# EveryVoiceTTS/EveryVoice

Measured on AMD Instinct MI355X. Metric: hifigan_v1_infer_audio_samples_per_sec, higher is better.
Workload: dtype bf16; 1 GPU; HiFiGAN-V1 generator inference, mel[32,80,768] -> wav[32,1,196608] per GPU, 1 replica(s), upstream N(0,0.01) init, weight norm folded; global_batch=32, frames=768, parallelism=replicas x1

## Files before the change

### everyvoice_amd/csrc/common.h

```cpp
#pragma once

#include <hip/hip_runtime.h>
#include <stdint.h>

#include <cstdio>
#include <cstdlib>
#include <string>

#include "evmi.h"

namespace evmi {

constexpr int kMaxDevices = 16;
inline int device_slot() {
  int d = 0;
  if (hipGetDevice(&d) != hipSuccess || d < 0 || d >= kMaxDevices) return 0;
  return d;
}


void set_error(const std::string& msg);
int fail(int code, const std::string& msg);

#define EVMI_HIP_CHECK(expr)                                                                   \
  do {                                                                                         \
    hipError_t _e = (expr);                                                                    \
    if (_e != hipSuccess) {                                                                    \
      return ::evmi::fail(EVMI_ERR_HIP, std::string(#expr) + ": " + hipGetErrorString(_e));    \
    }                                                                                          \
  } while (0)

#define EVMI_LAUNCH_CHECK(what)                                                                \
  do {                                                                                         \
    hipError_t _e = hipGetLastError();                                                         \
    if (_e != hipSuccess) {                                                                    \
      return ::evmi::fail(EVMI_ERR_HIP, std::string(what) + " launch: " + hipGetErrorString(_e)); \
    }                                                                                          \
  } while (0)

constexpr int kMaxLdsKernels = 256;
inline int ensure_dynamic_lds(const void* kernel, size_t bytes) {
  struct Record { const void* kernel; size_t bytes; };
  static thread_local Record records[kMaxDevices][kMaxLdsKernels];
  static thread_local int n_records[kMaxDevices] = {};
  int d = -1;
  if (hipGetDevice(&d) != hipSuccess || d >= kMaxDevices) d = -1;
  Record* r = nullptr;
  if (d >= 0) {
    for (int i = 0; i < n_records[d] && !r; ++i)
      if (records[d][i].kernel == kernel) r = &records[d][i];
    if (r && bytes <= r->bytes) return EVMI_OK;
  }
  const hipError_t e = hipFuncSetAttribute(kernel, hipFuncAttributeMaxDynamicSharedMemorySize, (int)bytes);
  if (e != hipSuccess)
    return fail(EVMI_ERR_HIP, "hipFuncSetAttribute(MaxDynamicSharedMemorySize, " + std::to_string(bytes) + "): " + hipGetErrorString(e));
  if (r) r->bytes = bytes;
  else if (d >= 0 && n_records[d] < kMaxLdsKernels) records[d][n_records[d]++] = Record{kernel, bytes};
  return EVMI_OK;
}

template <typename... Params, typename... Args>
inline int launch_with_lds(void (*kernel)(Params...), dim3 grid, dim3 block, size_t lds, hipStream_t stream, Args&&... args) {
  if (int rc = ensure_dynamic_lds((const void*)kernel, lds)) return rc;
  hipLaunchKernelGGL(kernel, grid, block, lds, stream, static_cast<Args&&>(args)...);
  return EVMI_OK;
}

inline int env_int(const char* name, int dflt) {
  const char* e = getenv(name);
  return e ? atoi(e) : dflt;
}
inline bool env_set(const char* name) { return getenv(name) != nullptr; }

typedef __bf16 bf16_t;
typedef __bf16 bf16x8 __attribute__((ext_vector_type(8)));
typedef __bf16 bf16x4 __attribute__((ext_vector_type(4)));
typedef float f32x16 __attribute__((ext_vector_type(16)));
typedef float f32x4 __attribute__((ext_vector_type(4)));
typedef unsigned int u32x4 __attribute__((ext_vector_type(4)));

__device__ __forceinline__ float lrelu(float v, float slope) { return v > 0.f ? v : v * slope; }

__device__ __forceinline__ u32x4 swap_quads_bf16(u32x4 d) {
  const auto r0 = __builtin_amdgcn_permlane32_swap(d[0], d[2], false, false);
  const auto r1 = __builtin_amdgcn_permlane32_swap(d[1], d[3], false, false);
  u32x4 o;
  o[0] = r0[0];
  o[2] = r0[1];
  o[1] = r1[0];
  o[3] = r1[1];
  return o;
}
__device__ __forceinline__ unsigned pack_bf16x2(float lo, float hi) {
  typedef __bf16 bf16x2_t __attribute__((ext_vector_type(2)));
  bf16x2_t pk;
  pk[0] = (bf16_t)lo;
  pk[1] = (bf16_t)hi;
  return __builtin_bit_cast(unsigned, pk);
}
__device__ __forceinline__ float bf16_lo(unsigned d) { return __builtin_bit_cast(float, d << 16); }
__device__ __forceinline__ float bf16_hi(unsigned d) { return __builtin_bit_cast(float, d & 0xffff0000u); }

__device__ __forceinline__ void lds_barrier() {
  asm volatile("s_waitcnt lgkmcnt(0)\n\ts_barrier" ::: "memory");
}

__device__ __forceinline__ void lds_dma_barrier() {
  asm volatile("s_waitcnt vmcnt(0)" ::: "memory");
  __syncthreads();
}

template <int MT, int NT, int KSTEPS, int NTAPS, int A_TAP_STRIDE, int A_MT_STRIDE, int B_NT_STRIDE, int PRIO = 0>
__device__ __forceinline__ void mma_tap_group(const bf16_t* __restrict__ Arow, const bf16_t* __restrict__ Brow,
                                              int b_tap_stride, f32x16 (&acc)[MT][NT]) {
  constexpr int N = NTAPS * KSTEPS;
  bf16x8 af[2][MT], bfr[2][NT];
  auto load = [&](int kk, int buf) {
    const int jj = kk / KSTEPS, ks = kk % KSTEPS;
#pragma unroll
    for (int mt = 0; mt < MT; ++mt)
      af[buf][mt] = *reinterpret_cast<const bf16x8*>(Arow + jj * A_TAP_STRIDE + mt * A_MT_STRIDE + ks * 16);
#pragma unroll
    for (int nt = 0; nt < NT; ++nt)
      bfr[buf][nt] = *reinterpret_cast<const bf16x8*>(Brow + jj * b_tap_stride + nt * B_NT_STRIDE + ks * 16);
  };
  load(0, 0);
#pragma unroll
  for (int kk = 0; kk < N; ++kk) {
    const int cur = kk & 1;
    if (kk + 1 < N) load(kk + 1, cur ^ 1);
    if (PRIO) __builtin_amdgcn_s_setprio(1);
#pragma unroll
    for (int mt = 0; mt < MT; ++mt)
#pragma unroll
      for (int nt = 0; nt < NT; ++nt)
        acc[mt][nt] = __builtin_amdgcn_mfma_f32_32x32x16_bf16(af[cur][mt], bfr[cur][nt], acc[mt][nt], 0, 0, 0);
    if (PRIO) __builtin_amdgcn_s_setprio(0);
  }
}

__device__ __forceinline__ bf16x4 lrelu4_bf16(f32x4 f, float slope) {
  const f32x4 m = f * slope;
  bf16x4 r;
#pragma unroll
  for (int e = 0; e < 4; ++e) r[e] = (bf16_t)fmaxf(f[e], m[e]);
  return r;
}
__device__ __forceinline__ bf16x8 lrelu8_bf16(bf16x8 x, float slope) {
  f32x4 lo, hi;
#pragma unroll
  for (int e = 0; e < 4; ++e) { lo[e] = (float)x[e]; hi[e] = (float)x[4 + e]; }
  const f32x4 ml = lo * slope, mh = hi * slope;
  bf16x8 r;
#pragma unroll
  for (int e = 0; e < 4; ++e) { r[e] = (bf16_t)fmaxf(lo[e], ml[e]); r[4 + e] = (bf16_t)fmaxf(hi[e], mh[e]); }
  return r;
}

inline uint16_t f32_to_bf16_bits(float f) {
  uint32_t u;
  __builtin_memcpy(&u, &f, 4);
  if ((u & 0x7fffffffu) > 0x7f800000u) return (uint16_t)((u >> 16) | 0x40);
  u += 0x7fffu + ((u >> 16) & 1u);
  return (uint16_t)(u >> 16);
}

__device__ __forceinline__ float ordered_sum_strided(const float* __restrict__ p, long long stride, int n, float acc = 0.f) {
  int s = 0;
  for (; s + 16 <= n; s += 16) {
    float v[16];
#pragma unroll
    for (int u = 0; u < 16; ++u) v[u] = p[(long long)(s + u) * stride];
#pragma unroll
    for (int u = 0; u < 16; ++u) acc += v[u];
  }
  for (; s < n; s += 8) {
    float v[8];
#pragma unroll
    for (int u = 0; u < 8; ++u) v[u] = p[(long long)min(s + u, n - 1) * stride];
#pragma unroll
    for (int u = 0; u < 8; ++u) acc = s + u < n ? acc + v[u] : acc;
  }
  return acc;
}


__device__ __forceinline__ float silu_grad(float z) {
#pragma clang fp contract(off)
  const float sg = 1.f / (1.f + expf(-z));
  return sg * (1.f + z * (1.f - sg));
}
__device__ __forceinline__ float silu_value(float v) {
#pragma clang fp contract(off)
  return v / (1.f + expf(-v));
}

struct SeedArg {
  unsigned long long value;
  const unsigned long long* base;
  __device__ __forceinline__ unsigned long long get() const { return base ? ((value + *base) & 0x7FFFFFFFFFFFFFFFull) : value; }
};

__device__ __forceinline__ unsigned dropout_hash(unsigned long long seed, unsigned j_lo, unsigned j_hi) {
  const unsigned k0 = (unsigned)seed * 0x9E3779B1u + 0x7F4A7C15u;
  unsigned k1 = (unsigned)(seed >> 32) ^ (k0 >> 15);
  k1 = k1 * 0x85EBCA6Bu + 0xC2B2AE35u;
  unsigned h = j_lo ^ k0;
  h += j_hi * 0x27D4EB2Fu;
  h ^= h >> 16;
  h *= 0x7FEB352Du;
  h ^= k1;
  h ^= h >> 15;
  h *= 0x846CA68Bu;
  h ^= h >> 16;
  return h;
}
__device__ __forceinline__ float dropout_u16(unsigned h, unsigned odd) { return (float)(odd ? h >> 16 : h & 0xFFFFu) * (1.0f / 65536.0f); }
__device__ __forceinline__ float uniform01(unsigned long long seed, unsigned long long i) {
  const unsigned long long j = i >> 1;
  return dropout_u16(dropout_hash(seed, (unsigned)j, (unsigned)(j >> 32)), (unsigned)i & 1u);
}
__device__ __forceinline__ void dropout_pair(unsigned long long seed, unsigned j, float& u_even, float& u_odd) {
  const unsigned h = dropout_hash(seed, j, 0u);
  u_even = dropout_u16(h, 0u);
  u_odd = dropout_u16(h, 1u);
}


__device__ __forceinline__ float wave_sum_dpp(float v) {
  v += __builtin_bit_cast(float, __builtin_amdgcn_mov_dpp(__builtin_bit_cast(int, v), 0xB1, 0xF, 0xF, true));
  v += __builtin_bit_cast(float, __builtin_amdgcn_mov_dpp(__builtin_bit_cast(int, v), 0x4E, 0xF, 0xF, true));
  v += __builtin_bit_cast(float, __builtin_amdgcn_mov_dpp(__builtin_bit_cast(int, v), 0x141, 0xF, 0xF, true));
  v += __builtin_bit_cast(float, __builtin_amdgcn_mov_dpp(__builtin_bit_cast(int, v), 0x140, 0xF, 0xF, true));
  const int b = __builtin_bit_cast(int, v);
  const float r0 = __builtin_bit_cast(float, __builtin_amdgcn_readlane(b, 0)), r1 = __builtin_bit_cast(float, __builtin_amdgcn_readlane(b, 16));
  const float r2 = __builtin_bit_cast(float, __builtin_amdgcn_readlane(b, 32)), r3 = __builtin_bit_cast(float, __builtin_amdgcn_readlane(b, 48));
  return (r0 + r1) + (r2 + r3);
}

template <int CTRL>
__device__ __forceinline__ double dpp_move_f64(double v) {
  const long long b = __builtin_bit_cast(long long, v);
  const int lo = __builtin_amdgcn_mov_dpp((int)(b & 0xFFFFFFFFll), CTRL, 0xF, 0xF, true);
  const int hi = __builtin_amdgcn_mov_dpp((int)(b >> 32), CTRL, 0xF, 0xF, true);
  return __builtin_bit_cast(double, ((long long)hi << 32) | (long long)(unsigned)lo);
}
__device__ __forceinline__ double wave_sum_dpp_f64(double v) {
  v += dpp_move_f64<0xB1>(v);
  v += dpp_move_f64<0x4E>(v);
  v += dpp_move_f64<0x141>(v);
  v += dpp_move_f64<0x140>(v);
  const long long b = __builtin_bit_cast(long long, v);
  const int lo = (int)(b & 0xFFFFFFFFll), hi = (int)(b >> 32);
  double r[4];
#pragma unroll
  for (int q = 0; q < 4; ++q) {
    const int l = __builtin_amdgcn_readlane(lo, 16 * q), h = __builtin_amdgcn_readlane(hi, 16 * q);
    r[q] = __builtin_bit_cast(double, ((long long)h << 32) | (long long)(unsigned)l);
  }
  return (r[0] + r[1]) + (r[2] + r[3]);
}

__device__ __forceinline__ void wait_vmcnt_le(int n) {
  n = __builtin_amdgcn_readfirstlane(n);
#define EVMI_VMCASE(N) case N: asm volatile("s_waitcnt vmcnt(" #N ")" ::: "memory"); break;
  switch (n) {
    EVMI_VMCASE(0) EVMI_VMCASE(1) EVMI_VMCASE(2) EVMI_VMCASE(3) EVMI_VMCASE(4) EVMI_VMCASE(5) EVMI_VMCASE(6)
    EVMI_VMCASE(7) EVMI_VMCASE(8) EVMI_VMCASE(9) EVMI_VMCASE(10) EVMI_VMCASE(11) EVMI_VMCASE(12) EVMI_VMCASE(13)
    EVMI_VMCASE(14) EVMI_VMCASE(15) EVMI_VMCASE(16) EVMI_VMCASE(17) EVMI_VMCASE(18) EVMI_VMCASE(19) EVMI_VMCASE(20)
    EVMI_VMCASE(21) EVMI_VMCASE(22) EVMI_VMCASE(23) EVMI_VMCASE(24) EVMI_VMCASE(25) EVMI_VMCASE(26) EVMI_VMCASE(27)
    EVMI_VMCASE(28) EVMI_VMCASE(29) EVMI_VMCASE(30) EVMI_VMCASE(31) EVMI_VMCASE(32) EVMI_VMCASE(33) EVMI_VMCASE(34)
    EVMI_VMCASE(35) EVMI_VMCASE(36) EVMI_VMCASE(37) EVMI_VMCASE(38) EVMI_VMCASE(39) EVMI_VMCASE(40) EVMI_VMCASE(41)
    EVMI_VMCASE(42) EVMI_VMCASE(43) EVMI_VMCASE(44) EVMI_VMCASE(45) EVMI_VMCASE(46) EVMI_VMCASE(47) EVMI_VMCASE(48)
    EVMI_VMCASE(49) EVMI_VMCASE(50) EVMI_VMCASE(51) EVMI_VMCASE(52) EVMI_VMCASE(53) EVMI_VMCASE(54) EVMI_VMCASE(55)
    EVMI_VMCASE(56) EVMI_VMCASE(57) EVMI_VMCASE(58) EVMI_VMCASE(59) EVMI_VMCASE(60) EVMI_VMCASE(61) EVMI_VMCASE(62)
    default: asm volatile("s_waitcnt vmcnt(63)" ::: "memory"); break;
  }
#undef EVMI_VMCASE
}


int launch_mha_fwd_bf16_plain(const float* qkv, const int* lens, float* out, float* lse_or_null, int B, int T, int D, int heads,
                              hipStream_t s);

}
```

### everyvoice_amd/csrc/conv_tc_dma_kernel.h

```cpp
#pragma once

#include <type_traits>

#include "conv_tc_mfma.h"

namespace evmi {

static __device__ __attribute__((aligned(128))) bf16_t g_conv_dma_zero_row[64];

typedef __attribute__((address_space(3))) void lds_void_t;
typedef __attribute__((address_space(1))) const void glb_void_t;
__device__ __forceinline__ void lds_dma_b128(const void* g, void* l) {
  __builtin_amdgcn_global_load_lds((glb_void_t*)g, (lds_void_t*)l, 16, 0, 0);
}

template <int CIN_, int KS_, int MAXDIL_, int DBG_ = 0, int VAR_ = 0, int WN_ = 4>
struct ConvDmaCfg {
  static constexpr int CIN = CIN_, KS = KS_, MAXDIL = MAXDIL_, DBG = DBG_, VAR = VAR_;
  static constexpr int KC = 64, BM = 128, WM = 2, WN = WN_, MT = 2, NT = 2, BN = WN * NT * 32;
  static constexpr int NTHREADS = WM * WN * 64, NWAVES = WM * WN;
  static constexpr int NCHUNK = CIN / KC, NSTEP = NCHUNK * KS;
  static constexpr int R_MAX = BN + (KS - 1) * MAXDIL;
  static constexpr int X_PIECES = (R_MAX + 7) / 8;
  static constexpr int X_BYTES = X_PIECES * 1024;
  static constexpr int A_PIECES = BM / 8;
  static constexpr int A_BYTES = A_PIECES * 1024;
  static constexpr int OS = BM + 8;
  static constexpr size_t LDS_MAIN = size_t(X_BYTES) + 2 * A_BYTES;
  static constexpr size_t LDS_OUT = size_t(BN) * OS * 2;
  static constexpr size_t LDS = LDS_MAIN > LDS_OUT ? LDS_MAIN : LDS_OUT;
  static constexpr int X_VEC_PER_THREAD = (X_PIECES * 64 + NTHREADS - 1) / NTHREADS;
  static_assert(CIN % KC == 0, "channel chunking");
  static_assert((WN == 4 ? 2 : 1) * LDS <= 160 * 1024, "two workgroups per CU (one for the 16-wave form)");
  static_assert(A_PIECES % NWAVES == 0 || NWAVES == 16, "weight pieces per wave");
};

template <class C>
__global__ __launch_bounds__(C::NTHREADS, 4) void conv_tc_dma_kernel(ConvTcArgs a) {
  static_assert(C::NWAVES == 2 || C::NWAVES == 4 || C::NWAVES == 8 || C::NWAVES == 16, "2, 4, 8 or 16 waves");
  extern __shared__ __attribute__((aligned(1024))) char smem[];
  char* Xs = smem;
  char* As = smem + C::X_BYTES;

  const int tid = threadIdx.x;
  const int lane = tid & 63;
  const int wave = __builtin_amdgcn_readfirstlane(tid >> 6);
  const int wm = wave / C::WN, wn = wave % C::WN;
  const int r0 = blockIdx.x * C::BN;
  const int b = blockIdx.y;
  const int mtile = blockIdx.z;
  const int m0 = mtile * C::BM;

  const bf16_t* __restrict__ xb = a.x + (long long)b * a.x_batch_stride;
  const bf16_t* __restrict__ wb = a.w + (long long)mtile * C::NSTEP * C::BM * C::KC;

  int n_stamp = 0;
  auto stamp = [&]() {
    if (C::DBG && a.timeline && blockIdx.x == 5 && blockIdx.y == 1 && blockIdx.z == 0 && lane == 0 && n_stamp < 120)
      a.timeline[wave * 128 + n_stamp++] = (long long)__builtin_readcyclecounter();
  };
  stamp();

  const int h = lane >> 5;
  const long long ob = (long long)b * a.out_batch_stride;
  long long flat_nt[C::NT];
  bool row_ok[C::NT];
#pragma unroll
  for (int nt = 0; nt < C::NT; ++nt) {
    const int r = r0 + wn * (C::NT * 32) + nt * 32 + (lane & 31);
    flat_nt[nt] = (long long)r * a.out_row_stride + m0 + wm * (C::MT * 32) + 8 * h + a.out_shift;
    row_ok[nt] = r < a.n_rows;
  }
  auto vec_index = [&](int nt, int co) -> long long {
    const long long f = flat_nt[nt] + co;
    return (row_ok[nt] && f >= 0 && f + 8 <= a.out_limit) ? f : -1;
  };
  auto swap_quads = [](u32x4 d) -> u32x4 { return swap_quads_bf16(d); };

  f32x16 acc[C::MT][C::NT];
#pragma unroll
  for (int mt = 0; mt < C::MT; ++mt)
#pragma unroll
    for (int q = 0; q < 4; ++q) {
      const f32x4 bv = *reinterpret_cast<const f32x4*>(a.bias + m0 + wm * (C::MT * 32) + mt * 32 + 8 * q + 4 * h);
#pragma unroll
      for (int nt = 0; nt < C::NT; ++nt)
#pragma unroll
        for (int i = 0; i < 4; ++i) acc[mt][nt][4 * q + i] = bv[i];
    }
  const int rows_needed = C::BN + (C::KS - 1) * a.dil;
  const int x_pieces = (rows_needed + 7) >> 3;
  const float pre = a.pre_slope;

  auto issue_a = [&](int step) {
    const bf16_t* src = wb + (long long)step * (C::BM * C::KC) + lane * 8;
    char* dst = As + (step & 1) * C::A_BYTES;
    if (C::VAR & 1024) {
      if (wave < C::NWAVES / 2) {
#pragma unroll
        for (int i = 0; i < 2 * C::A_PIECES / C::NWAVES; ++i) {
          const int p = wave + i * (C::NWAVES / 2);
          lds_dma_b128(src + p * 512, dst + p * 1024);
        }
      }
      return;
    }
#pragma unroll
    for (int i = 0; i < (C::A_PIECES + C::NWAVES - 1) / C::NWAVES; ++i) {
      const int p = wave + i * C::NWAVES;
      if (p < C::A_PIECES) lds_dma_b128(src + p * 512, dst + p * 1024);
    }
  };
  auto issue_x = [&](int chunk) {
    const int slot = lane & 7;
    for (int p = wave; p < x_pieces; p += C::NWAVES) {
      const int row = p * 8 + (lane >> 3);
      const int rr = r0 - a.pad + row;
      const int c8 = slot ^ ((row >> 1) & 7);
      const bf16_t* src = (row < rows_needed && rr >= 0 && rr < a.t_in) ? xb + (long long)rr * C::CIN + chunk * C::KC + c8 * 8
                                                                        : g_conv_dma_zero_row + slot * 8;
      lds_dma_b128(src, Xs + p * 1024);
    }
  };

  const int row_a = wm * (C::MT * 32) + (lane & 31);
  const int s_a = (row_a >> 1) & 7;
  int off_a[4];
#pragma unroll
  for (int ks = 0; ks < 4; ++ks) off_a[ks] = row_a * 128 + (((2 * ks + h) ^ s_a) << 4);

  auto mma_step = [&](const char* Ab, int tap, int next_step) {
    const int q = wn * (C::NT * 32) + (lane & 31) + tap * a.dil;
    const int s_b = (q >> 1) & 7;
    int off_b[4];
#pragma unroll
    for (int ks = 0; ks < 4; ++ks) off_b[ks] = q * 128 + (((2 * ks + h) ^ s_b) << 4);
    bf16x8 af[2][C::MT], bfr[2][C::NT];
    auto load = [&](int ks, int buf) {
#pragma unroll
      for (int mt = 0; mt < C::MT; ++mt) af[buf][mt] = *reinterpret_cast<const bf16x8*>(Ab + off_a[ks] + mt * (32 * 128));
#pragma unroll
      for (int nt = 0; nt < C::NT; ++nt) bfr[buf][nt] = *reinterpret_cast<const bf16x8*>(Xs + off_b[ks] + nt * (32 * 128));
    };
    load(0, 0);
#pragma unroll
    for (int ks = 0; ks < 4; ++ks) {
      const int cur = (C::VAR & 32) ? 0 : (ks & 1);
      if (ks + 1 < 4 && !(C::VAR & 32)) load(ks + 1, cur ^ 1);
      if ((C::VAR & 2048) && ks == 0 && next_step >= 0) issue_a(next_step);
      if (C::VAR & 2) __builtin_amdgcn_sched_barrier(0);
      if (C::VAR & 4) __builtin_amdgcn_s_setprio(1);
#pragma unroll
      for (int mt = 0; mt < C::MT; ++mt)
#pragma unroll
        for (int nt = 0; nt < C::NT; ++nt)
          acc[mt][nt] = __builtin_amdgcn_mfma_f32_32x32x16_bf16(af[cur][mt], bfr[cur][nt], acc[mt][nt], 0, 0, 0);
      if (C::VAR & 4) __builtin_amdgcn_s_setprio(0);
      if (C::VAR & 2) __builtin_amdgcn_sched_barrier(0);
    }
  };
  if ((C::VAR & 1) && wave >= C::NWAVES / 2) __builtin_amdgcn_s_setprio(1);

  issue_x(0);
  issue_a(0);
#pragma unroll 1
  for (int chunk = 0; chunk < C::NCHUNK; ++chunk) {
    if (chunk > 0 && !(C::VAR & 64)) {
      __syncthreads();
      issue_x(chunk);
    }
    if (pre != 1.f && !((C::VAR & 64) && chunk > 0)) {
      lds_dma_barrier();
#pragma unroll
      for (int i = 0; i < C::X_VEC_PER_THREAD; ++i) {
        const int v = tid + i * C::NTHREADS;
        if (v < x_pieces * 64) {
          bf16x8 val = *reinterpret_cast<const bf16x8*>(Xs + v * 16);
#pragma unroll
          for (int e = 0; e < 8; ++e) {
            const float f = (float)val[e];
            val[e] = (bf16_t)fmaxf(f, f * pre);
          }
          *reinterpret_cast<bf16x8*>(Xs + v * 16) = val;
        }
      }
    }
    stamp();
#pragma unroll 1
    for (int tap = 0; tap < C::KS; ++tap) {
      const int step = chunk * C::KS + tap;
      if (!(C::VAR & (16 | 256)) || step == 0) lds_dma_barrier();
      stamp();
      const bool more = step + 1 < C::NSTEP && !(C::VAR & (16 | 512));
      if (more && !(C::VAR & 2048)) issue_a(step + 1);
      mma_step(As + (step & 1) * C::A_BYTES, tap, (more && (C::VAR & 2048)) ? step + 1 : -1);
      stamp();
    }
  }

  if (C::VAR & 128) {
    float sacc = 0.f;
#pragma unroll
    for (int mt = 0; mt < C::MT; ++mt)
#pragma unroll
      for (int nt = 0; nt < C::NT; ++nt)
#pragma unroll
        for (int r = 0; r < 16; ++r) sacc += acc[mt][nt][r];
    if (sacc == 12345.678f) a.out[0] = (bf16_t)sacc;
    return;
  }
  stamp();
  if (a.res || a.mask) {
    __syncthreads();
    bf16_t* Os = reinterpret_cast<bf16_t*>(smem);
#pragma unroll
    for (int mt = 0; mt < C::MT; ++mt)
#pragma unroll
      for (int q = 0; q < 4; ++q) {
        const int c = wm * C::MT * 32 + mt * 32 + 8 * q + 4 * h;
#pragma unroll
        for (int nt = 0; nt < C::NT; ++nt) {
          const int n = wn * C::NT * 32 + nt * 32 + (lane & 31);
          bf16x4 pk;
#pragma unroll
          for (int i = 0; i < 4; ++i) pk[i] = (bf16_t)acc[mt][nt][4 * q + i];
          *reinterpret_cast<bf16x4*>(Os + n * C::OS + c) = pk;
        }
      }
    __syncthreads();
    const float scale = a.out_scale, post = a.post_slope;
    constexpr int VPR = C::BM / 8;
    constexpr int OPT = C::BN * VPR / C::NTHREADS;
    constexpr int EB = 4;
    static_assert(C::BN * VPR % C::NTHREADS == 0 && OPT % EB == 0, "epilogue tiling");
    auto flat_index = [&](int v) -> long long {
      const int n = v / VPR, c8 = v % VPR;
      const int r = r0 + n;
      const long long flat = (long long)r * a.out_row_stride + m0 + c8 * 8 + a.out_shift;
      return (r >= a.n_rows || flat < 0 || flat >= a.out_limit) ? -1 : flat;
    };
    const float mslope = a.mask_slope;
    auto body = [&](auto has_acc, auto has_res, auto has_mask) {
      constexpr bool ACC = decltype(has_acc)::value, RES = decltype(has_res)::value, MSK = decltype(has_mask)::value;
#pragma unroll
      for (int i0 = 0; i0 < OPT; i0 += EB) {
        bf16x8 rv[EB], pv[EB], mv[EB];
#pragma unroll
        for (int i = 0; i < EB; ++i) {
          const long long flat = flat_index(tid + (i0 + i) * C::NTHREADS);
          const long long safe = flat < 0 ? 0 : flat;
          if (RES) rv[i] = *reinterpret_cast<const bf16x8*>(a.res + ob + safe);
          if (ACC) pv[i] = *reinterpret_cast<const bf16x8*>(a.out + ob + safe);
          if (MSK) mv[i] = *reinterpret_cast<const bf16x8*>(a.mask + ob + safe);
        }
#pragma unroll
        for (int i = 0; i < EB; ++i) {
          const int v = tid + (i0 + i) * C::NTHREADS;
          const long long flat = flat_index(v);
          const int n = v / VPR, c8 = v % VPR;
          const bf16x8 o = *reinterpret_cast<const bf16x8*>(Os + n * C::OS + c8 * 8);
          float f[8];
#pragma unroll
          for (int e = 0; e < 8; ++e) f[e] = (float)o[e];
          if (MSK) {
#pragma unroll
            for (int e = 0; e < 8; ++e) f[e] = (float)mv[i][e] > 0.f ? f[e] : f[e] * mslope;
          }
          if (RES) {
#pragma unroll
            for (int e = 0; e < 8; ++e) f[e] += (float)rv[i][e];
          }
#pragma unroll
          for (int e = 0; e < 8; ++e) f[e] *= scale;
          if (ACC) {
#pragma unroll
            for (int e = 0; e < 8; ++e) f[e] += (float)pv[i][e];
          }
          bf16x8 res;
#pragma unroll
          for (int e = 0; e < 8; ++e) res[e] = (bf16_t)(post != 1.f ? lrelu(f[e], post) : f[e]);
          if (flat >= 0) *reinterpret_cast<bf16x8*>(a.out + ob + flat) = res;
        }
      }
    };
    using T_ = std::integral_constant<bool, true>;
    using F_ = std::integral_constant<bool, false>;
    if (a.mask) {
      if (a.res) body(F_{}, T_{}, T_{});
      else body(F_{}, F_{}, T_{});
    } else if (a.accumulate) body(T_{}, T_{}, F_{});
    else body(F_{}, T_{}, F_{});
  } else {
    const float scale = a.out_scale, post = a.post_slope;
    auto body = [&](auto has_acc) {
      constexpr bool ACC = decltype(has_acc)::value;
#pragma unroll
      for (int mt = 0; mt < C::MT; ++mt) {
        u32x4 pv[C::NT][2];
        if (ACC) {
#pragma unroll
          for (int nt = 0; nt < C::NT; ++nt)
#pragma unroll
            for (int p2 = 0; p2 < 2; ++p2) {
              const long long f = vec_index(nt, mt * 32 + 16 * p2);
              pv[nt][p2] = *reinterpret_cast<const u32x4*>(a.out + ob + (f < 0 ? 0 : f));
            }
        }
#pragma unroll
        for (int nt = 0; nt < C::NT; ++nt)
#pragma unroll
          for (int p2 = 0; p2 < 2; ++p2) {
            float f[8];
#pragma unroll
            for (int e = 0; e < 8; ++e) f[e] = acc[mt][nt][8 * p2 + e] * scale;
            if (ACC) {
              const u32x4 d = swap_quads(pv[nt][p2]);
#pragma unroll
              for (int w = 0; w < 4; ++w) {
                f[2 * w] += __builtin_bit_cast(float, d[w] << 16);
                f[2 * w + 1] += __builtin_bit_cast(float, d[w] & 0xffff0000u);
              }
            }
            u32x4 o;
#pragma unroll
            for (int w = 0; w < 4; ++w) {
              const float lo = post != 1.f ? lrelu(f[2 * w], post) : f[2 * w];
              const float hi = post != 1.f ? lrelu(f[2 * w + 1], post) : f[2 * w + 1];
              typedef __bf16 bf16x2_t __attribute__((ext_vector_type(2)));
              bf16x2_t pk;
              pk[0] = (bf16_t)lo;
              pk[1] = (bf16_t)hi;
              o[w] = __builtin_bit_cast(unsigned, pk);
            }
            o = swap_quads(o);
            const long long fo = vec_index(nt, mt * 32 + 16 * p2);
            if (fo >= 0) *reinterpret_cast<u32x4*>(a.out + ob + fo) = o;
          }
      }
    };
    if (a.accumulate) body(std::integral_constant<bool, true>{});
    else body(std::integral_constant<bool, false>{});
  }
  stamp();
}

template <class C>
static ConvTcLaunch make_conv_dma_launch(const char* name) {
  ConvTcLaunch l;
  l.kernel = conv_tc_dma_kernel<C>;
  l.bm = C::BM;
  l.bn = C::BN;
  l.kc = C::KC;
  l.threads = C::NTHREADS;
  l.lds_bytes = C::LDS;
  l.name = name;
  l.wlayout = 1;
  return l;
}

}
```

### everyvoice_amd/csrc/conv_tc_mfma.hip

```cpp
#include "conv_tc_dma_kernel.h"
#include "conv_tc_kernel.h"

namespace evmi {

struct ConvTcEntry {
  int c_in, ks, max_dil, kc;
  ConvTcLaunch launch;
};

template <class C>
static ConvTcEntry make_entry(const char* name) {
  ConvTcEntry e;
  e.c_in = C::CIN;
  e.ks = C::KS;
  e.max_dil = C::MAXDIL;
  e.kc = C::KC;
  e.launch = make_conv_tc_launch<C>(name);
  return e;
}

#define EVMI_CONV_TC_TABLE(X)                                                        \
                                                         \
  X(80, 80, 128, 128, 2, 2, 7, 1, 1)                                                 \
                          \
  X(512, 64, 128, 256, 2, 4, 2, 1, 1)                                                \
  X(256, 64, 128, 256, 2, 4, 2, 1, 1)                                                \
  X(128, 64, 128, 256, 2, 4, 2, 1, 1)                                                \
  X(64, 64, 64, 256, 1, 8, 2, 2, 1)                                                  \
                                 \
  X(256, 64, 128, 256, 2, 4, 3, 1, 5)                                                \
  X(256, 64, 128, 256, 2, 4, 7, 1, 5)                                                \
  X(256, 64, 128, 256, 2, 4, 11, 1, 5)                                               \
  X(128, 64, 128, 256, 2, 4, 3, 1, 5)                                                \
  X(128, 64, 128, 256, 2, 4, 7, 1, 5)                                                \
  X(128, 64, 128, 256, 2, 4, 11, 1, 5)                                               \
  X(64, 64, 64, 256, 1, 8, 3, 3, 5)                                                  \
  X(64, 64, 64, 256, 1, 8, 7, 1, 5)                                                  \
  X(64, 64, 64, 256, 1, 8, 11, 1, 5)                                                 \
  X(32, 32, 32, 512, 1, 8, 3, 3, 5)                                                  \
  X(32, 32, 32, 512, 1, 8, 7, 7, 5)                                                  \
  X(32, 32, 32, 512, 1, 8, 11, 11, 5)

static const ConvTcEntry* conv_tc_table(int* n) {
#define X(cin, kc, bm, bn, wm, wn, ks, taps, md)                                               \
  make_entry<ConvTcCfg<cin, kc, bm, bn, wm, wn, ks, taps, md>>(                                \
      "conv_tc_mfma<c" #cin ",k" #ks ",bm" #bm ",bn" #bn ",kc" #kc ",t" #taps ">"),
  static const ConvTcEntry table[] = {EVMI_CONV_TC_TABLE(X)};
#undef X
  *n = (int)(sizeof(table) / sizeof(table[0]));
  return table;
}

#define EVMI_CONV_DMA_TABLE(X) \
  X(512, 2, 1) X(256, 2, 1) X(128, 2, 1) X(256, 3, 5) X(256, 7, 5) X(256, 11, 5) X(128, 3, 5) X(128, 7, 5) X(128, 11, 5)

#define EVMI_CONV_DMA_NARROW_TABLE(X) X(256, 3, 5) X(256, 7, 5) X(256, 11, 5) X(128, 3, 5) X(128, 7, 5) X(128, 11, 5)

static const ConvTcEntry* conv_dma_table(int* n) {
#define X(cin, ks, md)                                                                          \
  ConvTcEntry{cin, ks, md, 64, make_conv_dma_launch<ConvDmaCfg<cin, ks, md>>("conv_tc_dma<c" #cin ",k" #ks ",bm128,bn256,kc64>")},
  static ConvTcEntry table[] = {EVMI_CONV_DMA_TABLE(X)};
#undef X
#define X(cin, ks, md)                                                                                                                   \
  ConvTcEntry{cin, ks, md, 64, make_conv_dma_launch<ConvDmaCfg<cin, ks, md, 0, 0, 2>>("conv_tc_dma<c" #cin ",k" #ks ",bm128,bn128,kc64>")},
  static const ConvTcEntry narrow[] = {EVMI_CONV_DMA_NARROW_TABLE(X)};
#undef X
  static const bool linked = [] {
    for (ConvTcEntry& e : table)
      for (const ConvTcEntry& nr : narrow)
        if (nr.c_in == e.c_in && nr.ks == e.ks && nr.max_dil == e.max_dil) e.launch.narrow = &nr.launch;
    return true;
  }();
  (void)linked;
  *n = (int)(sizeof(table) / sizeof(table[0]));
  return table;
}

const ConvTcLaunch* find_conv_tc(int c_in, int c_out, int ks, int dil) {
  static const bool use_dma = env_int("EVMI_CONV_DMA", 1) != 0;
  if (use_dma) {
    int nd = 0;
    const ConvTcEntry* d = conv_dma_table(&nd);
    for (int i = 0; i < nd; ++i)
      if (d[i].c_in == c_in && d[i].ks == ks && dil <= d[i].max_dil && c_out % d[i].launch.bm == 0) return &d[i].launch;
  }
  int n = 0;
  const ConvTcEntry* t = conv_tc_table(&n);
  for (int i = 0; i < n; ++i) {
    if (t[i].c_in == c_in && t[i].ks == ks && dil <= t[i].max_dil && c_out % t[i].launch.bm == 0)
      return &t[i].launch;
  }
  return nullptr;
}

int launch_conv_tc(const ConvTcLaunch* L, const ConvTcArgs& a, int B, hipStream_t stream) {
  static const int narrow_on = env_int("EVMI_CONV_NARROW", 1);
  if (narrow_on && !L->persistent && L->narrow && (long long)((a.n_rows + L->bn - 1) / L->bn) * B * (a.c_out / L->bm) < 256) L = L->narrow;
  dim3 grid((a.n_rows + L->bn - 1) / L->bn, B, a.c_out / L->bm);
  ConvTcArgs args = a;
  args.n_items = B;
  if (L->persistent) {
    const int dev_slot = device_slot();
    static thread_local int n_cu_dev[kMaxDevices] = {};
    if (!n_cu_dev[dev_slot]) {
      int dev = 0;
      hipDeviceProp_t prop;
      EVMI_HIP_CHECK(hipGetDevice(&dev));
      EVMI_HIP_CHECK(hipGetDeviceProperties(&prop, dev));
      n_cu_dev[dev_slot] = prop.multiProcessorCount > 0 ? prop.multiProcessorCount : 256;
    }
    const long long n_rb = (long long)B * grid.x;
    const long long total = (n_rb + 7) / 8 * 8 * grid.z;
    grid = dim3((unsigned)(total < n_cu_dev[dev_slot] ? total : n_cu_dev[dev_slot]), 1, 1);
  }
  if (int rc = launch_with_lds(L->kernel, grid, dim3(L->threads), L->lds_bytes, stream, args)) return rc;
  EVMI_LAUNCH_CHECK(L->name);
  return EVMI_OK;
}

}
```

Measured before the change: 371.4 million samples/s.

## Switch DMA conv kernel to 16x16x32 MFMA tiles with new LDS swizzle

Adds a 16x16x32 bf16 MFMA path to the DMA-fed conv kernel and makes it the default. The X-tile swizzle, fragment offsets, accumulator layout, bias init, epilogue mapping and quad swap (permlane16) are rewritten for the smaller tiles. A-fragment loads are pipelined across eight groups with a three-slot buffer. The aim is better MFMA issue efficiency and fewer accumulator registers per wave, at the cost of more LDS reads per FLOP and a riskier layout remap in the epilogue.

```diff
diff --git a/everyvoice_amd/csrc/common.h b/everyvoice_amd/csrc/common.h
--- a/everyvoice_amd/csrc/common.h
+++ b/everyvoice_amd/csrc/common.h
@@ -84,6 +84,16 @@
 __device__ __forceinline__ u32x4 swap_quads_bf16(u32x4 d) {
   const auto r0 = __builtin_amdgcn_permlane32_swap(d[0], d[2], false, false);
   const auto r1 = __builtin_amdgcn_permlane32_swap(d[1], d[3], false, false);
+  u32x4 o;
+  o[0] = r0[0];
+  o[2] = r0[1];
+  o[1] = r1[0];
+  o[3] = r1[1];
+  return o;
+}
+__device__ __forceinline__ u32x4 swap_quads16_bf16(u32x4 d) {
+  const auto r0 = __builtin_amdgcn_permlane16_swap(d[0], d[2], false, false);
+  const auto r1 = __builtin_amdgcn_permlane16_swap(d[1], d[3], false, false);
   u32x4 o;
   o[0] = r0[0];
   o[2] = r0[1];
diff --git a/everyvoice_amd/csrc/conv_tc_dma_kernel.h b/everyvoice_amd/csrc/conv_tc_dma_kernel.h
--- a/everyvoice_amd/csrc/conv_tc_dma_kernel.h
+++ b/everyvoice_amd/csrc/conv_tc_dma_kernel.h
@@ -3,6 +3,7 @@
 #include <type_traits>
 
 #include "conv_tc_mfma.h"
+#include "mfma16_layout.h"
 
 namespace evmi {
 
@@ -14,9 +15,10 @@
   __builtin_amdgcn_global_load_lds((glb_void_t*)g, (lds_void_t*)l, 16, 0, 0);
 }
 
-template <int CIN_, int KS_, int MAXDIL_, int DBG_ = 0, int VAR_ = 0, int WN_ = 4>
+template <int CIN_, int KS_, int MAXDIL_, int DBG_ = 0, int VAR_ = 0, int WN_ = 4, int MFMA_ = 16>
 struct ConvDmaCfg {
-  static constexpr int CIN = CIN_, KS = KS_, MAXDIL = MAXDIL_, DBG = DBG_, VAR = VAR_;
+  static constexpr int CIN = CIN_, KS = KS_, MAXDIL = MAXDIL_, DBG = DBG_, VAR = VAR_, MFMA = MFMA_;
+  static_assert(MFMA == 32 || MFMA == 16, "MFMA shape: 32 (32x32x16) or 16 (16x16x32)");
   static constexpr int KC = 64, BM = 128, WM = 2, WN = WN_, MT = 2, NT = 2, BN = WN * NT * 32;
   static constexpr int NTHREADS = WM * WN * 64, NWAVES = WM * WN;
   static constexpr int NCHUNK = CIN / KC, NSTEP = NCHUNK * KS;
@@ -61,33 +63,38 @@
   };
   stamp();
 
+  constexpr bool M16 = C::MFMA == 16;
+  constexpr int MTT = C::MT * 32 / C::MFMA, NTT = C::NT * 32 / C::MFMA;
   const int h = lane >> 5;
   const long long ob = (long long)b * a.out_batch_stride;
-  long long flat_nt[C::NT];
-  bool row_ok[C::NT];
-#pragma unroll
-  for (int nt = 0; nt < C::NT; ++nt) {
+  auto vec_index = [&](int nt, int co) -> long long {
     const int r = r0 + wn * (C::NT * 32) + nt * 32 + (lane & 31);
-    flat_nt[nt] = (long long)r * a.out_row_stride + m0 + wm * (C::MT * 32) + 8 * h + a.out_shift;
-    row_ok[nt] = r < a.n_rows;
+    const long long f = (long long)r * a.out_row_stride + m0 + wm * (C::MT * 32) + 8 * h + a.out_shift + co;
+    return (r < a.n_rows && f >= 0 && f + 8 <= a.out_limit) ? f : -1;
+  };
+  auto swap_quads = [](u32x4 d) -> u32x4 { return M16 ? swap_quads16_bf16(d) : swap_quads_bf16(d); };
+
+  using acc_t = std::conditional_t<M16, f32x4, f32x16>;
+  acc_t acc[MTT][NTT];
+  if constexpr (M16) {
+#pragma unroll
+    for (int mt = 0; mt < MTT; ++mt) {
+      const f32x4 bv = *reinterpret_cast<const f32x4*>(a.bias + m0 + wm * (C::MT * 32) + mt * 16 + mfma16::acc_channel(lane, 0));
+#pragma unroll
+      for (int nt = 0; nt < NTT; ++nt) acc[mt][nt] = bv;
+    }
+  } else {
+#pragma unroll
+    for (int mt = 0; mt < C::MT; ++mt)
+#pragma unroll
+      for (int q = 0; q < 4; ++q) {
+        const f32x4 bv = *reinterpret_cast<const f32x4*>(a.bias + m0 + wm * (C::MT * 32) + mt * 32 + 8 * q + 4 * h);
+#pragma unroll
+        for (int nt = 0; nt < C::NT; ++nt)
+#pragma unroll
+          for (int i = 0; i < 4; ++i) acc[mt][nt][4 * q + i] = bv[i];
+      }
   }
-  auto vec_index = [&](int nt, int co) -> long long {
-    const long long f = flat_nt[nt] + co;
-    return (row_ok[nt] && f >= 0 && f + 8 <= a.out_limit) ? f : -1;
-  };
-  auto swap_quads = [](u32x4 d) -> u32x4 { return swap_quads_bf16(d); };
-
-  f32x16 acc[C::MT][C::NT];
-#pragma unroll
-  for (int mt = 0; mt < C::MT; ++mt)
-#pragma unroll
-    for (int q = 0; q < 4; ++q) {
-      const f32x4 bv = *reinterpret_cast<const f32x4*>(a.bias + m0 + wm * (C::MT * 32) + mt * 32 + 8 * q + 4 * h);
-#pragma unroll
-      for (int nt = 0; nt < C::NT; ++nt)
-#pragma unroll
-        for (int i = 0; i < 4; ++i) acc[mt][nt][4 * q + i] = bv[i];
-    }
   const int rows_needed = C::BN + (C::KS - 1) * a.dil;
   const int x_pieces = (rows_needed + 7) >> 3;
   const float pre = a.pre_slope;
@@ -116,47 +123,76 @@
     for (int p = wave; p < x_pieces; p += C::NWAVES) {
       const int row = p * 8 + (lane >> 3);
       const int rr = r0 - a.pad + row;
-      const int c8 = slot ^ ((row >> 1) & 7);
+      const int c8 = slot ^ (M16 ? mfma16::x_swizzle(row) : (row >> 1) & 7);
       const bf16_t* src = (row < rows_needed && rr >= 0 && rr < a.t_in) ? xb + (long long)rr * C::CIN + chunk * C::KC + c8 * 8
                                                                         : g_conv_dma_zero_row + slot * 8;
       lds_dma_b128(src, Xs + p * 1024);
     }
   };
 
-  const int row_a = wm * (C::MT * 32) + (lane & 31);
+  const int row_a = wm * (C::MT * 32) + (lane & (C::MFMA - 1));
   const int s_a = (row_a >> 1) & 7;
-  int off_a[4];
-#pragma unroll
-  for (int ks = 0; ks < 4; ++ks) off_a[ks] = row_a * 128 + (((2 * ks + h) ^ s_a) << 4);
+  constexpr int NKS = M16 ? 2 : 4;
+  int off_a[NKS];
+#pragma unroll
+  for (int ks = 0; ks < NKS; ++ks)
+    off_a[ks] = M16 ? mfma16::frag_offset(row_a, mfma16::frag_vec(lane, ks), mfma16::w_swizzle(row_a)) : row_a * 128 + (((2 * ks + h) ^ s_a) << 4);
 
   auto mma_step = [&](const char* Ab, int tap, int next_step) {
-    const int q = wn * (C::NT * 32) + (lane & 31) + tap * a.dil;
-    const int s_b = (q >> 1) & 7;
-    int off_b[4];
-#pragma unroll
-    for (int ks = 0; ks < 4; ++ks) off_b[ks] = q * 128 + (((2 * ks + h) ^ s_b) << 4);
-    bf16x8 af[2][C::MT], bfr[2][C::NT];
-    auto load = [&](int ks, int buf) {
-#pragma unroll
-      for (int mt = 0; mt < C::MT; ++mt) af[buf][mt] = *reinterpret_cast<const bf16x8*>(Ab + off_a[ks] + mt * (32 * 128));
-#pragma unroll
-      for (int nt = 0; nt < C::NT; ++nt) bfr[buf][nt] = *reinterpret_cast<const bf16x8*>(Xs + off_b[ks] + nt * (32 * 128));
-    };
-    load(0, 0);
-#pragma unroll
-    for (int ks = 0; ks < 4; ++ks) {
-      const int cur = (C::VAR & 32) ? 0 : (ks & 1);
-      if (ks + 1 < 4 && !(C::VAR & 32)) load(ks + 1, cur ^ 1);
-      if ((C::VAR & 2048) && ks == 0 && next_step >= 0) issue_a(next_step);
-      if (C::VAR & 2) __builtin_amdgcn_sched_barrier(0);
-      if (C::VAR & 4) __builtin_amdgcn_s_setprio(1);
-#pragma unroll
-      for (int mt = 0; mt < C::MT; ++mt)
-#pragma unroll
-        for (int nt = 0; nt < C::NT; ++nt)
-          acc[mt][nt] = __builtin_amdgcn_mfma_f32_32x32x16_bf16(af[cur][mt], bfr[cur][nt], acc[mt][nt], 0, 0, 0);
-      if (C::VAR & 4) __builtin_amdgcn_s_setprio(0);
-      if (C::VAR & 2) __builtin_amdgcn_sched_barrier(0);
+    if constexpr (M16) {
+      const int q = wn * (C::NT * 32) + (lane & 15) + tap * a.dil;
+      const int s_b = mfma16::x_swizzle(q);
+      int off_b[2];
+#pragma unroll
+      for (int s = 0; s < 2; ++s) off_b[s] = mfma16::frag_offset(q, mfma16::frag_vec(lane, s), s_b);
+      bf16x8 af[3], bfr[2][NTT];
+      auto load_a = [&](int grp) {
+        af[grp % 3] = *reinterpret_cast<const bf16x8*>(Ab + off_a[grp >> 2] + (grp & 3) * (16 * 128));
+      };
+      auto load_b = [&](int s, int nt) { bfr[s][nt] = *reinterpret_cast<const bf16x8*>(Xs + off_b[s] + nt * (16 * 128)); };
+      load_a(0);
+#pragma unroll
+      for (int nt = 0; nt < NTT; ++nt) load_b(0, nt);
+      load_a(1);
+#pragma unroll
+      for (int grp = 0; grp < 8; ++grp) {
+        if (grp + 2 < 8) load_a(grp + 2);
+        if (grp < 4) load_b(1, grp);
+        if (C::VAR & 2) __builtin_amdgcn_sched_barrier(0);
+#pragma unroll
+        for (int nt = 0; nt < NTT; ++nt)
+          acc[grp & 3][nt] = __builtin_amdgcn_mfma_f32_16x16x32_bf16(af[grp % 3], bfr[grp >> 2][nt], acc[grp & 3][nt], 0, 0, 0);
+        if (C::VAR & 2) __builtin_amdgcn_sched_barrier(0);
+      }
+    } else {
+      const int q = wn * (C::NT * 32) + (lane & 31) + tap * a.dil;
+      const int s_b = (q >> 1) & 7;
+      int off_b[4];
+#pragma unroll
+      for (int ks = 0; ks < 4; ++ks) off_b[ks] = q * 128 + (((2 * ks + h) ^ s_b) << 4);
+      bf16x8 af[2][C::MT], bfr[2][C::NT];
+      auto load = [&](int ks, int buf) {
+#pragma unroll
+        for (int mt = 0; mt < C::MT; ++mt) af[buf][mt] = *reinterpret_cast<const bf16x8*>(Ab + off_a[ks] + mt * (32 * 128));
+#pragma unroll
+        for (int nt = 0; nt < C::NT; ++nt) bfr[buf][nt] = *reinterpret_cast<const bf16x8*>(Xs + off_b[ks] + nt * (32 * 128));
+      };
+      load(0, 0);
+#pragma unroll
+      for (int ks = 0; ks < 4; ++ks) {
+        const int cur = (C::VAR & 32) ? 0 : (ks & 1);
+        if (ks + 1 < 4 && !(C::VAR & 32)) load(ks + 1, cur ^ 1);
+        if ((C::VAR & 2048) && ks == 0 && next_step >= 0) issue_a(next_step);
+        if (C::VAR & 2) __builtin_amdgcn_sched_barrier(0);
+        if (C::VAR & 4) __builtin_amdgcn_s_setprio(1);
+#pragma unroll
+        for (int mt = 0; mt < C::MT; ++mt)
+#pragma unroll
+          for (int nt = 0; nt < C::NT; ++nt)
+            acc[mt][nt] = __builtin_amdgcn_mfma_f32_32x32x16_bf16(af[cur][mt], bfr[cur][nt], acc[mt][nt], 0, 0, 0);
+        if (C::VAR & 4) __builtin_amdgcn_s_setprio(0);
+        if (C::VAR & 2) __builtin_amdgcn_sched_barrier(0);
+      }
     }
   };
   if ((C::VAR & 1) && wave >= C::NWAVES / 2) __builtin_amdgcn_s_setprio(1);
@@ -201,11 +237,11 @@
   if (C::VAR & 128) {
     float sacc = 0.f;
 #pragma unroll
-    for (int mt = 0; mt < C::MT; ++mt)
-#pragma unroll
-      for (int nt = 0; nt < C::NT; ++nt)
-#pragma unroll
-        for (int r = 0; r < 16; ++r) sacc += acc[mt][nt][r];
+    for (int mt = 0; mt < MTT; ++mt)
+#pragma unroll
+      for (int nt = 0; nt < NTT; ++nt)
+#pragma unroll
+        for (int r = 0; r < (M16 ? 4 : 16); ++r) sacc += acc[mt][nt][r];
     if (sacc == 12345.678f) a.out[0] = (bf16_t)sacc;
     return;
   }
@@ -213,20 +249,35 @@
   if (a.res || a.mask) {
     __syncthreads();
     bf16_t* Os = reinterpret_cast<bf16_t*>(smem);
-#pragma unroll
-    for (int mt = 0; mt < C::MT; ++mt)
-#pragma unroll
-      for (int q = 0; q < 4; ++q) {
-        const int c = wm * C::MT * 32 + mt * 32 + 8 * q + 4 * h;
-#pragma unroll
-        for (int nt = 0; nt < C::NT; ++nt) {
-          const int n = wn * C::NT * 32 + nt * 32 + (lane & 31);
+    if constexpr (M16) {
+#pragma unroll
+      for (int mt = 0; mt < MTT; ++mt) {
+        const int c = wm * C::MT * 32 + mt * 16 + mfma16::acc_channel(lane, 0);
+#pragma unroll
+        for (int nt = 0; nt < NTT; ++nt) {
+          const int n = wn * C::NT * 32 + nt * 16 + mfma16::acc_row(lane);
           bf16x4 pk;
 #pragma unroll
-          for (int i = 0; i < 4; ++i) pk[i] = (bf16_t)acc[mt][nt][4 * q + i];
+          for (int i = 0; i < 4; ++i) pk[i] = (bf16_t)acc[mt][nt][i];
           *reinterpret_cast<bf16x4*>(Os + n * C::OS + c) = pk;
         }
       }
+    } else {
+#pragma unroll
+      for (int mt = 0; mt < C::MT; ++mt)
+#pragma unroll
+        for (int q = 0; q < 4; ++q) {
+          const int c = wm * C::MT * 32 + mt * 32 + 8 * q + 4 * h;
+#pragma unroll
+          for (int nt = 0; nt < C::NT; ++nt) {
+            const int n = wn * C::NT * 32 + nt * 32 + (lane & 31);
+            bf16x4 pk;
+#pragma unroll
+            for (int i = 0; i < 4; ++i) pk[i] = (bf16_t)acc[mt][nt][4 * q + i];
+            *reinterpret_cast<bf16x4*>(Os + n * C::OS + c) = pk;
+          }
+        }
+    }
     __syncthreads();
     const float scale = a.out_scale, post = a.post_slope;
     constexpr int VPR = C::BM / 8;
@@ -312,7 +363,10 @@
           for (int p2 = 0; p2 < 2; ++p2) {
             float f[8];
 #pragma unroll
-            for (int e = 0; e < 8; ++e) f[e] = acc[mt][nt][8 * p2 + e] * scale;
+            for (int e = 0; e < 8; ++e) {
+              if constexpr (M16) f[e] = acc[2 * mt + p2][2 * nt + (e >> 2)][e & 3] * scale;
+              else f[e] = acc[mt][nt][8 * p2 + e] * scale;
+            }
             if (ACC) {
               const u32x4 d = swap_quads(pv[nt][p2]);
 #pragma unroll
diff --git a/everyvoice_amd/csrc/conv_tc_mfma.hip b/everyvoice_amd/csrc/conv_tc_mfma.hip
--- a/everyvoice_amd/csrc/conv_tc_mfma.hip
+++ b/everyvoice_amd/csrc/conv_tc_mfma.hip
@@ -56,13 +56,14 @@
 
 #define EVMI_CONV_DMA_NARROW_TABLE(X) X(256, 3, 5) X(256, 7, 5) X(256, 11, 5) X(128, 3, 5) X(128, 7, 5) X(128, 11, 5)
 
+template <int MFMA>
 static const ConvTcEntry* conv_dma_table(int* n) {
 #define X(cin, ks, md)                                                                          \
-  ConvTcEntry{cin, ks, md, 64, make_conv_dma_launch<ConvDmaCfg<cin, ks, md>>("conv_tc_dma<c" #cin ",k" #ks ",bm128,bn256,kc64>")},
+  ConvTcEntry{cin, ks, md, 64, make_conv_dma_launch<ConvDmaCfg<cin, ks, md, 0, 0, 4, MFMA>>("conv_tc_dma<c" #cin ",k" #ks ",bm128,bn256,kc64>")},
   static ConvTcEntry table[] = {EVMI_CONV_DMA_TABLE(X)};
 #undef X
 #define X(cin, ks, md)                                                                                                                   \
-  ConvTcEntry{cin, ks, md, 64, make_conv_dma_launch<ConvDmaCfg<cin, ks, md, 0, 0, 2>>("conv_tc_dma<c" #cin ",k" #ks ",bm128,bn128,kc64>")},
+  ConvTcEntry{cin, ks, md, 64, make_conv_dma_launch<ConvDmaCfg<cin, ks, md, 0, 0, 2, MFMA>>("conv_tc_dma<c" #cin ",k" #ks ",bm128,bn128,kc64>")},
   static const ConvTcEntry narrow[] = {EVMI_CONV_DMA_NARROW_TABLE(X)};
 #undef X
   static const bool linked = [] {
@@ -79,8 +80,9 @@
 const ConvTcLaunch* find_conv_tc(int c_in, int c_out, int ks, int dil) {
   static const bool use_dma = env_int("EVMI_CONV_DMA", 1) != 0;
   if (use_dma) {
+    static const int mfma = env_int("EVMI_CONV_MFMA", 16);
     int nd = 0;
-    const ConvTcEntry* d = conv_dma_table(&nd);
+    const ConvTcEntry* d = mfma == 32 ? conv_dma_table<32>(&nd) : conv_dma_table<16>(&nd);
     for (int i = 0; i < nd; ++i)
       if (d[i].c_in == c_in && d[i].ks == ks && dil <= d[i].max_dil && c_out % d[i].launch.bm == 0) return &d[i].launch;
   }
diff --git a/everyvoice_amd/csrc/mfma16_layout.h b/everyvoice_amd/csrc/mfma16_layout.h
--- /dev/null
+++ b/everyvoice_amd/csrc/mfma16_layout.h
@@ -0,0 +1,24 @@
+#pragma once
+
+namespace evmi {
+namespace mfma16 {
+
+#if defined(__HIPCC__)
+#define EVMI_HD __host__ __device__ __forceinline__
+#else
+#define EVMI_HD inline
+#endif
+
+EVMI_HD constexpr int x_swizzle(int row) { return row & 6; }
+EVMI_HD constexpr int w_swizzle(int row) { return (row >> 1) & 7; }
+EVMI_HD constexpr int frag_vec(int lane, int s) { return (lane >> 4) + 4 * s; }
+EVMI_HD constexpr int frag_offset(int row, int vec, int swz) { return row * 128 + ((vec ^ swz) << 4); }
+EVMI_HD constexpr int acc_row(int lane) { return lane & 15; }
+EVMI_HD constexpr int acc_channel(int lane, int i) { return 4 * (lane >> 4) + i; }
+EVMI_HD constexpr int swapped_tile(int lane) { return (lane >> 4) & 1; }
+EVMI_HD constexpr int swapped_channel(int lane) { return 8 * (lane >> 5); }
+
+#undef EVMI_HD
+
+}
+}
```

After: 385.2 million samples/s (median of 6 runs). 1.04x the previous value.
